# hrz2000/CustomNeRF

Measured on AMD Instinct MI355X. Metric: training rays/s, higher is better.
Workload: dtype f16

## Files before the change

customnerf_amd/_lib.py:

```python
import ctypes as C
import os

import torch

_HERE = os.path.dirname(os.path.abspath(__file__))
LIB_PATH = os.path.join(_HERE, "libcustomnerf_hip.so")
ABI_VERSION = 8

vp, u32, u64, f32, i32 = C.c_void_p, C.c_uint32, C.c_uint64, C.c_float, C.c_int

SIGNATURES = {
    "cnerf_abi_version": [],
    "cnerf_profile_stage_events": [vp, u32],
    "cnerf_near_far_from_aabb": [vp, vp, vp, u32, f32, vp, vp, vp],
    "cnerf_sph_from_ray": [vp, vp, f32, u32, vp, vp],
    "cnerf_morton3D": [vp, u32, vp, vp],
    "cnerf_morton3D_invert": [vp, u32, vp, vp],
    "cnerf_packbits": [vp, u32, f32, vp, vp],
    "cnerf_march_rays_train": [vp, vp, vp, f32, f32, u32, u32, u32, u32, u32, vp, vp, vp, vp, vp, vp, vp, vp, vp],
    "cnerf_march_rays_train_count": [vp, vp, vp, f32, f32, u32, u32, u32, u32, vp, vp, vp, vp, vp, vp],
    "cnerf_march_rays_train_write": [vp, vp, vp, f32, f32, u32, u32, u32, u32, u32, vp, vp, vp, vp, vp, vp, vp, vp],
    "cnerf_march_rays_train_count_hits": [vp, vp, vp, f32, f32, u32, u32, u32, u32, vp, vp, vp, vp, vp, vp, vp],
    "cnerf_march_rays_train_write_hits": [vp, vp, f32, f32, u32, u32, u32, u32, u32, vp, vp, vp, vp, vp, vp, vp, vp],
    "cnerf_composite_rays_train_forward": [vp, vp, vp, vp, u32, u32, f32, vp, vp, vp, u32, vp],
# ... 85 lines not shown
    "cnerf_mesh_atlas_sized_measure": [vp, u32, vp, u32, vp, u64, vp, vp],
    "cnerf_mesh_atlas_sized_layout": [vp, u32, vp, vp, vp],
    "cnerf_mesh_atlas_sized_plan": [u32, u32, u32, vp, vp, u64, vp, vp, u32, vp],
    "cnerf_mesh_atlas_sized_uvs": [u32, u32, vp, vp, vp, u32, vp],
    "cnerf_mesh_atlas_sized_points": [vp, vp, u32, vp, u32, u32, vp, vp, u64, u32, u32, vp, vp, vp, u32, vp],
    "cnerf_mesh_atlas_sized_tspace": [vp, vp, u32, vp, u32, u32, vp, vp, u64, vp, u32, u32, vp, u32, vp, vp, u32, vp],
    "cnerf_mesh_atlas_sized_store": [u32, u32, vp, vp, u64, u32, u32, vp, u32, vp, vp, vp, vp],
    "cnerf_mesh_atlas_sized_fill": [u32, u32, vp, vp, vp],
    "cnerf_mesh_atlas_proj_workspace_bytes": [u32, u32, u32, vp],
    "cnerf_mesh_atlas_proj_charts": [vp, vp, u32, vp, u32, u32, vp, u64, vp, vp, vp, u32, vp, u32, vp],
    "cnerf_mesh_atlas_proj_pack": [vp, u32, u32, u32, vp, vp],
    "cnerf_mesh_atlas_proj_raster": [vp, u32, vp, u32, u32, u32, C.c_double, vp, u32, vp, u64, vp, vp, u32, vp, vp, vp, vp],
    "cnerf_mesh_atlas_proj_points": [vp, vp, u32, vp, u32, u32, vp, u64, u32, u32, vp, vp, vp, u32, vp],
    "cnerf_mesh_atlas_proj_tspace": [vp, vp, u32, vp, u32, u32, vp, u64, vp, u32, u32, vp, u32, vp, vp, u32, vp],
    "cnerf_mesh_atlas_proj_store": [u32, u32, u32, vp, u64, u32, u32, vp, u32, vp, vp, vp],
    "cnerf_mesh_atlas_proj_fill": [u32, u32, u32, vp, u64, vp, vp, vp, vp],
    "cnerf_mesh_tangent_workspace_bytes": [u32, u32, vp],
    "cnerf_mesh_tangent_weld": [vp, vp, u32, u32, vp, u64, vp, vp, u32, vp, u32, vp],
    "cnerf_mesh_tangent_frames": [vp, vp, vp, vp, u32, u32, vp, u64, vp, u32, vp],
    "cnerf_mesh_tangent_vertices": [vp, vp, vp, vp, vp, vp, vp, u32, u32, u32, vp, u64, vp, vp, vp, vp, vp, vp],
    "cnerf_mesh_raster_workspace_bytes": [u32, u32, u32, u32, vp],
    "cnerf_mesh_raster_visibility": [vp, u32, vp, u32, vp, f32, f32, f32, f32, u32, u32, i32, f32, i32, vp, u64, vp, vp, vp, vp, vp],
    "cnerf_mesh_raster_shade": [vp, vp, vp, u32, u32, vp, u32, u32, i32, vp, vp, vp, u32, vp, vp, f32, f32, vp, vp, vp, vp],
    "cnerf_tsdf_integrate": [vp, u32, u32, u32, vp, vp, f32, vp, vp, u32, u32, u32, vp, f32, f32, f32, f32, i32, f32, i32, vp],
    "cnerf_tsdf_finalize": [vp, u32, u32, u32, f32, vp, vp, vp],
    "cnerf_tsdf_face_keep": [vp, u32, u32, u32, vp, vp, vp, u32, vp, u32, vp, vp],
    "cnerf_view_colors_accumulate": [vp, vp, u32, vp, vp, vp, u32, u32, u32, vp, f32, f32, f32, f32, i32, f32, i32, f32, f32, i32, vp, vp, vp],
    "cnerf_view_colors_resolve": [vp, vp, u32, vp, vp, vp, vp, vp],
    "cnerf_mesh_holes_workspace_bytes": [u32, u32, vp],
    "cnerf_mesh_topology": [vp, u32, u32, vp, u64, vp, vp],
    "cnerf_mesh_topology_loops": [u32, u32, vp, u64, vp, u32, vp],
    "cnerf_mesh_holes_count": [vp, u32, u32, u32, vp, u64, vp, vp],
    "cnerf_mesh_holes_emit": [vp, vp, u32, vp, u32, u32, vp, u64, vp, vp, vp, u32, u32, vp],
    "cnerf_mesh_bvh_workspace_bytes": [u32, u32, vp],
    "cnerf_mesh_bvh_build": [vp, u32, vp, u32, vp, u64, vp, vp],
    "cnerf_mesh_bvh_closest": [vp, u64, u32, u32, vp, u32, vp, vp, vp, vp, vp, vp],
    "cnerf_mesh_sample_workspace_bytes": [u32, vp],
    "cnerf_mesh_sample_count": [vp, u32, vp, u32, f32, vp, u64, vp, vp],
    "cnerf_mesh_sample_emit": [vp, u32, vp, u32, f32, vp, u64, vp, vp, vp, vp, u64, vp],
    "cnerf_mesh_bvh_raycast": [vp, u64, u32, u32, vp, vp, u32, f32, f32, vp, vp, i32, vp, vp, vp, vp, vp],
    "cnerf_mesh_bvh_occluded": [vp, u64, u32, u32, vp, vp, u32, f32, f32, vp, vp, i32, vp, vp, vp],
    "cnerf_mesh_bvh_project": [vp, u64, u32, u32, vp, vp, vp, vp, u32, f32, vp, vp, vp, vp, vp, vp, vp, vp],
    "cnerf_mesh_winding_workspace_bytes": [u32, u32, vp],
    "cnerf_mesh_winding_build": [vp, u64, u32, u32, vp, u64, vp],
    "cnerf_mesh_winding_query": [vp, u64, u32, u32, vp, u64, vp, u32, f32, vp, vp, vp],
    "cnerf_mesh_bvh_signed_distance": [vp, u64, u32, u32, vp, u64, vp, u32, f32, vp, vp, vp, vp, vp],
    "cnerf_image_metrics_workspace_bytes": [u32, u32, u32, u32, vp],
    "cnerf_image_metrics": [vp, vp, vp, u32, u32, u32, u32, i32, i32, vp, vp, vp, vp],
    "cnerf_ssim_grad_workspace_bytes": [u32, u32, u32, u32, vp],
    "cnerf_ssim_grad": [vp, vp, vp, u32, u32, u32, u32, i32, vp, vp, vp, vp],
    "cnerf_sd_gemm": [vp, vp, u64, vp],
    "cnerf_sd_gemm_workspace_bytes": [vp, vp],
    "cnerf_sd_gemm_serves_ln": [vp, vp],
    "cnerf_sd_groupnorm_forward": [vp, vp, vp, u32, u32, u32, u32, f32, i32, vp, i32, vp, vp],
    "cnerf_sd_groupnorm_backward": [vp, vp, vp, vp, u32, u32, u32, u32, f32, i32, vp, vp, vp, vp],
    "cnerf_sd_groupnorm_backward_ex": [vp, vp, vp, vp, u32, u32, u32, u32, f32, i32, vp, vp, i32, vp, vp, vp],
    "cnerf_sd_layernorm_forward": [vp, vp, vp, u32, u32, f32, vp, vp],
    "cnerf_sd_softmax_forward": [vp, u64, u32, u32, vp],
    "cnerf_sd_softmax_backward": [vp, vp, u64, u32, u32, vp],
    "cnerf_sd_attention": [vp, vp, vp, vp, u32, u32, u32, u32, u32, u32, u64, u32, u64, u32, u64, u32, u64, i32, vp],
    "cnerf_sd_attention_v": [vp, vp, vp, vp, u32, u32, u32, u32, u32, u32, u64, u32, u64, u32, u64, u32, u64, i32, vp],
    "cnerf_sd_geglu": [vp, u64, u32, vp, vp],
    "cnerf_sd_transpose": [vp, vp, u32, u32, u32, u32, u32, u64, u64, vp],
    "cnerf_sd_image_to_vae_input": [vp, u32, u32, u32, u32, u32, vp, vp],
    "cnerf_sd_image_to_vae_input_backward": [vp, u32, u32, u32, u32, u32, vp, vp],
    "cnerf_sd_clip_preprocess": [vp, u32, u32, u32, u32, vp, vp, vp, vp],
    "cnerf_sd_patchify": [vp, u32, u32, u32, vp, vp],
    "cnerf_sd_timestep_embedding": [vp, u32, u32, vp, vp],
    "cnerf_sd_add_noise": [vp, vp, f32, u32, vp, vp],
    "cnerf_sd_sds_grad": [vp, u32, vp, f32, f32, f32, u32, vp, vp],
    "cnerf_sd_decoder_input": [vp, u32, u32, f32, vp, vp, vp],
    "cnerf_sd_decoder_output": [vp, u32, u32, u32, vp, vp, vp],
    "cnerf_sd_ddim_step": [vp, u32, vp, f32, f32, f32, i32, u32, u32, vp, vp, vp, vp],
    "cnerf_edit_ray_images": [vp, u32, u32, vp, vp, vp, vp],
    "cnerf_edit_ray_images_backward": [vp, vp, vp, u32, u32, vp, vp],
    "cnerf_edit_l1_loss": [vp, vp, u32, f32, vp, vp, vp],
    "cnerf_edit_sds_loss": [vp, vp, u32, vp, vp, vp],
    "cnerf_edit_scale_by_scalar": [vp, vp, f32, u32, vp, vp],
    "cnerf_sd_sample_latents": [vp, vp, u32, u32, f32, vp, vp],
    "cnerf_sd_sample_latents_backward": [vp, vp, vp, u32, u32, f32, vp, vp],
    "cnerf_set_floats": [vp, vp, u32, vp],
    "cnerf_sd_add": [vp, vp, u64, vp, vp],
    "cnerf_sd_silu": [vp, u64, vp, vp],
    "cnerf_sd_concat": [vp, vp, u64, u32, u32, vp, vp],
    "cnerf_sd_concat_gn": [vp, vp, u64, u32, u32, vp, vp, u32, u32, vp],
}


class SdGemmDesc(C.Structure):
    _fields_ = [("A", vp), ("B", vp), ("C", vp), ("C32", vp), ("bias", vp), ("bias_rows", vp), ("residual", vp),
                ("M", u32), ("N", u32), ("K", u32), ("lda", u32), ("ldb", u32), ("ldc", u32), ("ldr", u32),
                ("rows_per_bias_row", u32), ("ld_bias_rows", u32), ("alpha", f32), ("act", C.c_int32), ("batch_outer", u32), ("batch_inner", u32),
                ("sa_o", u64), ("sa_i", u64), ("sb_o", u64), ("sb_i", u64), ("sc_o", u64), ("sc_i", u64),
                ("mode", C.c_int32), ("Cin", u32), ("H_in", u32), ("W_in", u32), ("H_out", u32), ("W_out", u32),
                ("KH", u32), ("KW", u32), ("stride", u32), ("pad_t", u32), ("pad_l", u32), ("ups", u32), ("tstride", u32),
                ("gn_sums", vp), ("gn_groups", u32), ("gn_rows", u32),
                ("ln_out", vp), ("ln_gamma", vp), ("ln_beta", vp), ("ln_eps", f32)]

ADAM_MAX_JOBS = 8


class AdamJobs(C.Structure):
    _fields_ = [("p", vp * ADAM_MAX_JOBS), ("g", vp * ADAM_MAX_JOBS), ("m", vp * ADAM_MAX_JOBS), ("v", vp * ADAM_MAX_JOBS), ("p_half", vp * ADAM_MAX_JOBS),
                ("n", u64 * ADAM_MAX_JOBS), ("lr", f32 * ADAM_MAX_JOBS), ("n_jobs", u32)]


# ... 115 lines not shown
```

customnerf_amd/csrc/sd_gemm.hip:

```cpp
#include "common.h"
#include "../../include/customnerf_sd.h"
#include "sd_gn_fix.h"

typedef _Float16 sd_h8 __attribute__((ext_vector_type(8)));
typedef float sd_f16v __attribute__((ext_vector_type(16)));
typedef float sd_f4 __attribute__((ext_vector_type(4)));

#define SG_BM 128
#define SG_BK 64
#define SG_LDK (SG_BK + 8)
#define SG_THREADS 256

__host__ __device__ __forceinline__ int sg_rho(int r, int hi) { return (r & 3) + 8 * (r >> 2) + 4 * hi; }
__host__ __device__ constexpr uint32_t sg_stage_halfs(int bn) { return (SG_BM + bn) * SG_LDK; }
__host__ __device__ constexpr uint32_t sg_lds_bytes(int bn) {
    const uint32_t stages = 2 * sg_stage_halfs(bn) * 2, ctile = SG_BM * (bn + 4) * 4;
    return stages > ctile ? stages : ctile;
}
__host__ __device__ constexpr uint32_t sg_lds_bytes_glds(int bn) {
    const uint32_t stages = 2 * (SG_BM + bn) * SG_BK * 2, ctile = SG_BM * (bn + 4) * 4;
    return stages > ctile ? stages : ctile;
}

__device__ __forceinline__ float sg_act(float v, int act) {
    if (act == 1) return v * __builtin_amdgcn_rcpf(1.0f + __expf(-v));
    if (act == 2) return 0.5f * v * (1.0f + erff(v * 0.70710678118654752f));
    if (act == 3) return v * __builtin_amdgcn_rcpf(1.0f + __expf(-1.702f * v));
    return v;
}

__device__ __forceinline__ bool sg_coord(int32_t num, uint32_t tstride, uint32_t ups, uint32_t n_in, uint32_t &out) {
    if (num < 0) return false;
    if (tstride == 2) {
        if (num & 1) return false;
        num >>= 1;
    }
    if (ups == 2) num >>= 1;
    out = (uint32_t)num;
    return out < n_in;
}

template <int BM, int BN, int NTHREADS, bool SPLIT>
__device__ __forceinline__ void sg_epilogue_phase2(const CnerfSdGemm &g, const float *ct, long long (*gn_lds)[36][2], uint32_t tid, uint32_t m0, uint32_t n0,
                                                   uint32_t zo, uint32_t zi, uint32_t split, float *__restrict__ partial) {
    constexpr uint32_t LDC = BN + 4;
    constexpr int SG_EPI_THREADS = NTHREADS;
    const bool do_gn = !SPLIT && g.gn_sums != nullptr;
    constexpr int GI = 4;
    const uint32_t gn_cg = do_gn ? g.N / g.gn_groups : 1u;
    const uint32_t gn_g0 = n0 / gn_cg, gn_i0 = do_gn ? m0 / g.gn_rows : 0u;
    if (do_gn) {
        for (uint32_t i = tid; i < GI * 36 * 2; i += SG_EPI_THREADS) (&gn_lds[0][0][0])[i] = 0;
        __syncthreads();
    }
    float gs[2][2] = {{0.0f, 0.0f}, {0.0f, 0.0f}};
// ... 122 lines not shown
            if (full && ((g.ldc | n) & 7) == 0 && ((((uintptr_t)C) & 15) == 0)) {
                sd_h8 o;
#pragma unroll
                for (int e = 0; e < 8; e++) o[e] = (_Float16)v[e];
                *reinterpret_cast<sd_h8 *>(cp) = o;
            } else {
#pragma unroll
                for (int e = 0; e < 8; e++)
                    if (INSIDE || n + e < g.N) cp[e] = (_Float16)v[e];
            }
        }
        if (C32) {
            float *cp = C32 + (size_t)m * ldc32 + n;
#pragma unroll
            for (int e = 0; e < 8; e++)
                if (INSIDE || n + e < g.N) cp[e] = v[e];
        }
    }
    };
    const bool inside = m0 + BM <= g.M && n0 + BN <= g.N;
    if (!gn3) {
        if (inside) phase2(std::true_type{}, std::false_type{});
        else phase2(std::false_type{}, std::false_type{});
    } else phase2(std::false_type{}, std::true_type{});
    if (do_gn) {
        if (gn_img != 0xFFFFFFFFu) {
            const uint32_t gl = (n0 + (tid % CPR) * 8) / gn_cg - gn_g0;
            gn_add(&gn_lds[gn_img - gn_i0][gl][0], gs[0][0]);
            gn_add(&gn_lds[gn_img - gn_i0][gl][1], gs[0][1]);
            gn_add(&gn_lds[gn_img - gn_i0][gl + 1][0], gs[1][0]);
            gn_add(&gn_lds[gn_img - gn_i0][gl + 1][1], gs[1][1]);
            if (gn3) {
                gn_add(&gn_lds[gn_img - gn_i0][gl + 2][0], gs3[0]);
                gn_add(&gn_lds[gn_img - gn_i0][gl + 2][1], gs3[1]);
            }
        }
        __syncthreads();
        const uint32_t n_img = g.M / g.gn_rows;
        for (uint32_t i = tid; i < GI * 36; i += SG_EPI_THREADS) {
            const uint32_t im = i / 36, gl = i % 36, img = gn_i0 + im, grp = gn_g0 + gl;
            const long long a = gn_lds[im][gl][0], b2 = gn_lds[im][gl][1];
            if (img < n_img && grp < g.gn_groups) {
                long long *dst = reinterpret_cast<long long *>(g.gn_sums) + ((size_t)img * g.gn_groups + grp) * 2;
                gn_add_fixed(dst, a);
                gn_add_fixed(dst + 1, b2);
            }
        }
    }
}

__device__ __forceinline__ uint32_t sg_swz(uint32_t row, uint32_t chunk) { return chunk ^ ((row >> 1) & 7u); }

template <int AMODE, int NT, bool SPLIT, bool GLDS = false, bool SIMPLE = false>
__global__ void __launch_bounds__(SG_THREADS) k_sd_gemm(const CnerfSdGemm g, float *__restrict__ partial, uint32_t k_tiles_per_split) {
    constexpr int BN = 64 * NT;
    constexpr int MT = 2, BM = SG_BM;
    constexpr int CB = BN * 8 / SG_THREADS;
    constexpr uint32_t STAGE = sg_stage_halfs(BN);
    extern __shared__ __attribute__((aligned(16))) unsigned char sg_lds[];
    _Float16 *lds = reinterpret_cast<_Float16 *>(sg_lds);
    const uint32_t tid = threadIdx.x, lane = tid & 63, wave = tid >> 6, hi = lane >> 5, li = lane & 31;
    const uint32_t wm = wave >> 1, wn = wave & 1;
    const uint32_t m0 = blockIdx.x * BM, n0 = blockIdx.y * BN;
    uint32_t z = 0, split = 0;
    if (SPLIT) split = blockIdx.z; else z = blockIdx.z;
    const uint32_t zo = z / g.batch_inner, zi = z - zo * g.batch_inner;
    const _Float16 *A = reinterpret_cast<const _Float16 *>(g.A) + g.sa_o * zo + g.sa_i * zi;
    const _Float16 *B = reinterpret_cast<const _Float16 *>(g.B) + g.sb_o * zo + g.sb_i * zi;

    const uint32_t arow = tid >> 1, ak = (tid & 1) * 32;
    const uint32_t brow = tid / (8 / CB), bk = (tid % (8 / CB)) * CB * 8;
    const _Float16 *abase;
    int32_t oh_s = 0, ow_s = 0;
    bool a_valid;
    {
        const uint32_t m = m0 + arow;
        a_valid = m < g.M;
        if (AMODE == 0) abase = A + (size_t)m * g.lda;
        else {
            const uint32_t hw = g.H_out * g.W_out;
            const uint32_t img = m / hw, rem = m - img * hw, oh = rem / g.W_out, ow = rem - oh * g.W_out;
            abase = A + (size_t)img * g.H_in * g.W_in * g.Cin;
            oh_s = (int32_t)(oh * g.stride) - (int32_t)g.pad_t;
            ow_s = (int32_t)(ow * g.stride) - (int32_t)g.pad_l;
        }
    }
    const uint32_t nrow = n0 + brow;
    const bool b_valid = nrow < g.N;
    const _Float16 *bbase = B + (size_t)nrow * g.ldb;

    const uint32_t n_ktiles = (g.K + SG_BK - 1) / SG_BK;
    uint32_t kt0 = 0, kt1 = n_ktiles;
    if (SPLIT) { kt0 = split * k_tiles_per_split; kt1 = min(kt0 + k_tiles_per_split, n_ktiles); }

    uint32_t t_kh = 0, t_kw = 0, t_c0 = 0;
    if (AMODE == 2) {
        const uint32_t tap = (kt0 * SG_BK) / g.Cin;
        t_c0 = kt0 * SG_BK - tap * g.Cin;
        t_kh = tap / g.KW;
        t_kw = tap - t_kh * g.KW;
    }

    sd_f16v acc[MT][NT];
#pragma unroll
    for (int i = 0; i < MT; i++)
#pragma unroll
        for (int j = 0; j < NT; j++)
#pragma unroll
            for (int r = 0; r < 16; r++) acc[i][j][r] = 0.0f;

    if constexpr (!GLDS) {
        uint4 sa[4], sb[CB];
        auto fetch = [&](uint32_t kt) __attribute__((always_inline)) {
            const uint32_t k = kt * SG_BK;
            if (AMODE == 0) {
    #pragma unroll
                for (int c = 0; c < 4; c++) sa[c] = (a_valid && k + ak + 8 * c < g.K) ? *reinterpret_cast<const uint4 *>(abase + k + ak + 8 * c) : make_uint4(0, 0, 0, 0);
            } else if (AMODE == 2) {
// ... 38 lines not shown
        __syncthreads();
        for (uint32_t kt = kt0; kt < kt1; kt++) {
            const uint32_t stage = (kt - kt0) & 1;
            if (kt + 1 < kt1) fetch(kt + 1);
            const _Float16 *sA = lds + stage * STAGE, *sB = sA + SG_BM * SG_LDK;
    #pragma unroll
            for (int s = 0; s < SG_BK / 16; s++) {
                sd_h8 a[2], b[NT];
    #pragma unroll
                for (int i = 0; i < 2; i++) a[i] = *reinterpret_cast<const sd_h8 *>(sA + (wm * 64 + i * 32 + li) * SG_LDK + s * 16 + 8 * hi);
    #pragma unroll
                for (int j = 0; j < NT; j++) b[j] = *reinterpret_cast<const sd_h8 *>(sB + (wn * 32 * NT + j * 32 + li) * SG_LDK + s * 16 + 8 * hi);
    #pragma unroll
                for (int i = 0; i < 2; i++)
    #pragma unroll
                    for (int j = 0; j < NT; j++) acc[i][j] = __builtin_amdgcn_mfma_f32_32x32x16_f16(a[i], b[j], acc[i][j], 0, 0, 0);
            }
            if (kt + 1 < kt1) commit(stage ^ 1);
            __syncthreads();
        }


    } else {
        constexpr uint32_t GSTAGE = (BM + BN) * SG_BK * 2;
        constexpr int RA = BM / 32;
        constexpr int RB = BN / 32;
        const uint32_t grow = tid >> 3, gch = tid & 7u;
        constexpr uint32_t OOB = 0xFFFFFF00u;
        const uint32_t a_batch = AMODE == 0 ? 1u : g.M / (g.H_out * g.W_out);
        const uint32_t a_bytes = AMODE == 0 ? (uint32_t)(((size_t)(g.M - 1) * g.lda + g.K) * 2) : (uint32_t)((size_t)a_batch * g.H_in * g.W_in * g.Cin * 2);
        const uint32_t b_bytes = (uint32_t)(((size_t)(g.N - 1) * g.ldb + g.K) * 2);
        const __amdgpu_buffer_rsrc_t rsA = __builtin_amdgcn_make_buffer_rsrc(const_cast<_Float16 *>(A), 0, a_bytes, 0x00020000);
        const __amdgpu_buffer_rsrc_t rsB = __builtin_amdgcn_make_buffer_rsrc(const_cast<_Float16 *>(B), 0, b_bytes, 0x00020000);
        constexpr bool simple = SIMPLE;
        const uint32_t wave_u = __builtin_amdgcn_readfirstlane(wave);
        uint32_t a_off[RA];
        int32_t a_oh[RA], a_ow[RA];
        bool a_ok[RA];
        const uint32_t a_sc0 = sg_swz(grow, gch) * 8;
#pragma unroll
        for (int r = 0; r < RA; r++) {
            const uint32_t row = 32 * r + grow, m = m0 + row;
            a_ok[r] = m < g.M;
            a_oh[r] = a_ow[r] = 0;
            const uint32_t mm = a_ok[r] ? m : 0;
            if (AMODE == 0) a_off[r] = (mm * g.lda + a_sc0) * 2;
            else {
                const uint32_t hw = g.H_out * g.W_out;
                const uint32_t img = mm / hw, rem = mm - img * hw, oh = rem / g.W_out, ow = rem - oh * g.W_out;
                a_oh[r] = (int32_t)(oh * g.stride) - (int32_t)g.pad_t;
                a_ow[r] = (int32_t)(ow * g.stride) - (int32_t)g.pad_l;
                a_off[r] = ((img * g.H_in + (uint32_t)a_oh[r]) * g.W_in + (uint32_t)a_ow[r]) * g.Cin * 2 + a_sc0 * 2;
                if (!simple) a_off[r] = img * g.H_in * g.W_in * g.Cin * 2 + a_sc0 * 2;
            }
        }
        uint32_t b_off[RB];
#pragma unroll
        for (int r = 0; r < RB; r++) {
            const uint32_t row = 32 * r + grow, n = n0 + row;
            b_off[r] = n < g.N ? (n * g.ldb + sg_swz(row, gch) * 8) * 2 : OOB;
        }
        uint32_t i_k = 0, i_tap = 0;
        unsigned char *i_sA = sg_lds, *i_sB = sg_lds;
        bool i_kin = true;
        auto issue_begin = [&](uint32_t kt, uint32_t stage) __attribute__((always_inline)) {
            i_k = kt * SG_BK;
            i_sA = sg_lds + (size_t)stage * GSTAGE;
            i_sB = i_sA + BM * SG_BK * 2;
            i_kin = i_k + a_sc0 < g.K;
            i_tap = AMODE == 2 ? ((t_kh * g.W_in + t_kw) * g.Cin + t_c0) * 2 : i_k * 2;
        };
        auto issue_round = [&](int q) __attribute__((always_inline)) {
            if (q < RA) {
                const int r = q;
                uint32_t voff;
                if (AMODE == 0) {
                    voff = (a_off[r] + i_tap) | ((a_ok[r] && i_kin) ? 0u : OOB);
                } else if (simple) {
                    const bool ok = a_ok[r] && (uint32_t)(a_oh[r] + (int32_t)t_kh) < g.H_in && (uint32_t)(a_ow[r] + (int32_t)t_kw) < g.W_in;
                    voff = (a_off[r] + i_tap) | (ok ? 0u : OOB);
                } else {
                    uint32_t ih = 0, iw = 0;
                    const bool ok = a_ok[r] && sg_coord(a_oh[r] + (int32_t)t_kh, g.tstride, g.ups, g.H_in, ih) &&
                                    sg_coord(a_ow[r] + (int32_t)t_kw, g.tstride, g.ups, g.W_in, iw);
                    voff = ok ? a_off[r] + ((ih * g.W_in + iw) * g.Cin + t_c0) * 2 : OOB;
                }
                __builtin_amdgcn_raw_ptr_buffer_load_lds(rsA, (__attribute__((address_space(3))) void *)(i_sA + (32 * r + 8 * wave_u) * 128), 16, voff, 0, 0, 0);
            } else {
                const int r = q - RA;
                const uint32_t voff = b_off[r] | (i_kin ? 0u : OOB);
                __builtin_amdgcn_raw_ptr_buffer_load_lds(rsB, (__attribute__((address_space(3))) void *)(i_sB + (32 * r + 8 * wave_u) * 128), 16, voff, i_k * 2, 0, 0);
            }
        };
        auto issue_end = [&]() __attribute__((always_inline)) {
            if (AMODE == 2) {
                t_c0 += SG_BK;
                if (t_c0 >= g.Cin) {
                    t_c0 = 0;
                    if (++t_kw == g.KW) { t_kw = 0; ++t_kh; }
                }
            }
        };
        auto issue = [&](uint32_t kt, uint32_t stage) __attribute__((always_inline)) {
            issue_begin(kt, stage);
#pragma unroll
            for (int q = 0; q < RA + RB; q++) issue_round(q);
            issue_end();
        };
        uint32_t a_rd[MT][4], b_rd[NT][4];
#pragma unroll
        for (int s2 = 0; s2 < 4; s2++) {
#pragma unroll
            for (int i = 0; i < MT; i++) {
                const uint32_t row = wm * 32 * MT + i * 32 + li;
                a_rd[i][s2] = row * 128 + sg_swz(row, 2 * s2 + hi) * 16;
            }
#pragma unroll
            for (int j = 0; j < NT; j++) {
                const uint32_t row = wn * 32 * NT + j * 32 + li;
                b_rd[j][s2] = row * 128 + sg_swz(row, 2 * s2 + hi) * 16;
            }
        }
        if (kt0 < kt1) issue(kt0, 0);
        asm volatile("s_waitcnt vmcnt(0)" ::: "memory");
        __syncthreads();
        for (uint32_t kt = kt0; kt < kt1; kt++) {
            const uint32_t stage = (kt - kt0) & 1;
            if (kt + 1 < kt1) issue(kt + 1, stage ^ 1);
            const unsigned char *sA = sg_lds + (size_t)stage * GSTAGE, *sB = sA + BM * SG_BK * 2;
            sd_h8 a[2][MT], b[2][NT];
// ... 399 lines not shown
        }
    }
    const float mean = cn_wave_sum(sum) / (float)g.N;
    float sq = 0.0f;
#pragma unroll
    for (int c = 0; c < CPL; c++)
        if (lane + 64 * c < nchunks) {
#pragma unroll
            for (int e = 0; e < 8; e++) { const float d = v[c][e] - mean; sq += d * d; }
        }
    const float rstd = rsqrtf(cn_wave_sum(sq) / (float)g.N + g.ln_eps);
#pragma unroll
    for (int c = 0; c < CPL; c++) {
        const uint32_t col = lane + 64 * c;
        if (col < nchunks) {
            sd_h8 o;
#pragma unroll
            for (int e = 0; e < 8; e++) o[e] = (_Float16)((v[c][e] - mean) * rstd * g.ln_gamma[col * 8 + e] + g.ln_beta[col * 8 + e]);
            *reinterpret_cast<sd_h8 *>(reinterpret_cast<_Float16 *>(g.ln_out) + (size_t)m * g.N + col * 8) = o;
        }
    }
}

static bool sg_ln_admissible(const CnerfSdGemm *g) {
    return g->ln_out && g->ln_gamma && g->ln_beta && g->C && !g->C32 && !g->gn_sums && g->act != 4 && (g->N & 7) == 0 && g->N <= 2048 && (g->ldc & 7) == 0 &&
           (!g->residual || (g->ldr & 7) == 0) && g->batch_outer * g->batch_inner == 1 &&
           ((((uintptr_t)g->C) | ((uintptr_t)g->ln_out) | ((uintptr_t)g->residual)) & 15) == 0;
}

static int sg_check(const CnerfSdGemm *g) {
    if (!g) return CNERF_ENULL;
    if (!g->A || !g->B || (!g->C && !g->C32)) return CNERF_ENULL;
    if (g->M == 0 || g->N == 0 || g->K == 0 || (g->K & 7) || (g->ldb & 7)) return CNERF_EINVAL;
    if (g->batch_outer == 0 || g->batch_inner == 0) return CNERF_EINVAL;
    if (g->act < 0 || g->act > 4) return CNERF_EINVAL;
    if (g->act == 4 && ((g->N & 7) || g->residual || g->C32 || !g->C || g->gn_sums)) return CNERF_EINVAL;
    if (g->bias_rows && g->rows_per_bias_row == 0) return CNERF_EINVAL;
    if (g->gn_sums && (g->gn_groups == 0 || g->N % g->gn_groups || g->N / g->gn_groups < 4 || g->gn_rows < 64 || g->M % g->gn_rows ||
                       g->batch_outer * g->batch_inner != 1))
        return CNERF_EINVAL;
    if ((((uintptr_t)g->A) | ((uintptr_t)g->B)) & 15) return CNERF_EINVAL;
    if (g->mode == 0) {
        if (g->lda & 7) return CNERF_EINVAL;
    } else if (g->mode == 1) {
        if (g->Cin == 0 || (g->Cin & 7) || g->KH == 0 || g->KW == 0 || g->K != g->KH * g->KW * g->Cin) return CNERF_EINVAL;
        if (g->H_out == 0 || g->W_out == 0 || g->M % (g->H_out * g->W_out)) return CNERF_EINVAL;
        if (g->ups < 1 || g->ups > 2 || g->tstride < 1 || g->tstride > 2 || g->stride == 0) return CNERF_EINVAL;
        if (g->batch_outer * g->batch_inner != 1) return CNERF_EINVAL;
    } else return CNERF_EINVAL;
    return CNERF_OK;
}

struct SgPlan { int nt; uint32_t splits, kps; };
static int sg_env(const char *name) { return cn_tune_env(name, 0); }
static SgPlan sg_plan(const CnerfSdGemm *g) {
    const uint32_t n_ktiles = cn_div_up(g->K, SG_BK);
    const uint32_t batch = g->batch_outer * g->batch_inner;
    static const int force_nt = sg_env("CNERF_SG_NT"), force_sp = sg_env("CNERF_SG_SPLITS");
    SgPlan best = {1, 1, n_ktiles};
    double best_cost = 1e30;
    for (int nt = 1; nt <= 2; nt++) {
        if (force_nt && nt != force_nt) continue;
        const uint32_t tiles = cn_div_up(g->M, SG_BM) * cn_div_up(g->N, 64 * nt) * batch;
        const double t_k = nt == 1 ? 1.0 : 1.5;
        const uint32_t max_sp = batch != 1 ? 1 : 32;
        for (uint32_t sp = 1; sp <= max_sp; sp++) {
            if (force_sp && sp != (uint32_t)force_sp && !(batch != 1 && sp == 1)) continue;
            const uint32_t kps = cn_div_up(n_ktiles, sp);
            if (sp > 1 && (kps < 8 || cn_div_up(n_ktiles, kps) != sp)) continue;
            const uint64_t blocks = (uint64_t)tiles * sp;
            const double rounds = (double)((blocks + 511) / 512);
            double cost = rounds * (kps + 8.0) * t_k;
            if (blocks < 256) cost *= 0.6 + 0.4 * (double)blocks / 256.0;
            if (sp > 1) cost += 3.0 + 2.0 * (double)g->M * g->N * 4.0 * sp / 4.0e6;
            if (cost < best_cost) { best_cost = cost; best = {nt, sp, kps}; }
        }
    }
    return best;
}
static int sg_pick_nt(const CnerfSdGemm *g) { return sg_plan(g).nt; }
static uint32_t sg_splits(const CnerfSdGemm *g, int nt, uint32_t &k_tiles_per_split) {
    (void)nt;
    const SgPlan p = sg_plan(g);
    k_tiles_per_split = p.kps;
    return p.splits;
}

static bool sg_glds_fits(const CnerfSdGemm *g) {
    const uint64_t lim = 0xFFFFFF00ull - 4096;
    const uint64_t a_bytes = g->mode == 0 ? ((uint64_t)(g->M - 1) * g->lda + g->K) * 2
                                          : (uint64_t)(g->M / (g->H_out * g->W_out)) * g->H_in * g->W_in * g->Cin * 2;
    const uint64_t b_bytes = ((uint64_t)(g->N - 1) * g->ldb + g->K) * 2;
    return a_bytes < lim && b_bytes < lim;
}
static bool sg_use_glds(const CnerfSdGemm *g) {
    static const int v = cn_tune_env("CNERF_SG_GLDS", 1);
    return v != 0 && sg_glds_fits(g);
}

#ifdef CNERF_TUNING
static bool sg_use_big(const CnerfSdGemm *g, const SgPlan &plan) {
    static const int on = cn_tune_env("CNERF_SG_BIG", 0);
    static const int min_tiles = cn_tune_env("CNERF_SG_BIG_TILES", 224), min_k = cn_tune_env("CNERF_SG_BIG_K", 512);
    if (!on || plan.splits > 1 || !sg_use_glds(g)) return false;
    if (g->mode != 0 && (g->Cin % SG_BK) != 0) return false;
    if (g->gn_sums && g->gn_rows < 128) return false;
    if (g->K < (uint32_t)min_k || (g->N % SGB_BN) > 0 && (g->N % SGB_BN) <= 64 && g->N < 1024) return false;
    const uint64_t tiles = (uint64_t)cn_div_up(g->M, SGB_BM) * cn_div_up(g->N, SGB_BN) * g->batch_outer * g->batch_inner;
    return tiles >= (uint64_t)min_tiles;
}

template <int SCHED>
static void sgb_launch_s(const CnerfSdGemm *g, hipStream_t st) {
    const dim3 grid(cn_div_up(g->M, SGB_BM), cn_div_up(g->N, SGB_BN), g->batch_outer * g->batch_inner);
    static bool attr_set = false;
    if (!attr_set) {
        (void)hipFuncSetAttribute(reinterpret_cast<const void *>(&k_sd_gemm_big<0, false, SCHED>), hipFuncAttributeMaxDynamicSharedMemorySize, sgb_lds_bytes());
        (void)hipFuncSetAttribute(reinterpret_cast<const void *>(&k_sd_gemm_big<2, false, SCHED>), hipFuncAttributeMaxDynamicSharedMemorySize, sgb_lds_bytes());
        (void)hipFuncSetAttribute(reinterpret_cast<const void *>(&k_sd_gemm_big<2, true, SCHED>), hipFuncAttributeMaxDynamicSharedMemorySize, sgb_lds_bytes());
        attr_set = true;
    }
    if (g->mode == 0) hipLaunchKernelGGL((k_sd_gemm_big<0, false, SCHED>), grid, dim3(SGB_THREADS), sgb_lds_bytes(), st, *g);
    else if (g->tstride == 1 && g->ups == 1) hipLaunchKernelGGL((k_sd_gemm_big<2, true, SCHED>), grid, dim3(SGB_THREADS), sgb_lds_bytes(), st, *g);
    else hipLaunchKernelGGL((k_sd_gemm_big<2, false, SCHED>), grid, dim3(SGB_THREADS), sgb_lds_bytes(), st, *g);
}
static void sgb_launch(const CnerfSdGemm *g, hipStream_t st) {
    static const int sched = cn_tune_env("CNERF_SGB_SCHED", 2);
    if (sched == 0) { sgb_launch_s<0>(g, st); return; }
    if (sched == 1) { sgb_launch_s<1>(g, st); return; }
    sgb_launch_s<2>(g, st);
}
#endif

template <int AMODE, int NT, bool SPLIT, bool GLDS, bool SIMPLE = false>
static void sg_launch_g(const CnerfSdGemm *g, dim3 grid, hipStream_t st, float *partial, uint32_t kps) {
    if constexpr (GLDS && AMODE == 2 && !SIMPLE) {
        if (g->tstride == 1 && g->ups == 1) { sg_launch_g<AMODE, NT, SPLIT, GLDS, true>(g, grid, st, partial, kps); return; }
    }
    static bool attr_set = false;
    auto kern = k_sd_gemm<AMODE, NT, SPLIT, GLDS, SIMPLE>;
    const uint32_t lds_bytes = GLDS ? sg_lds_bytes_glds(64 * NT) : sg_lds_bytes(64 * NT);
    if (!attr_set) {
        (void)hipFuncSetAttribute(reinterpret_cast<const void *>(kern), hipFuncAttributeMaxDynamicSharedMemorySize, lds_bytes);
        attr_set = true;
    }
    hipLaunchKernelGGL(kern, grid, dim3(SG_THREADS), lds_bytes, st, *g, partial, kps);
}

template <int AMODE, int NT, bool SPLIT>
static void sg_launch(const CnerfSdGemm *g, dim3 grid, hipStream_t st, float *partial, uint32_t kps) {
    if constexpr (AMODE != 1) {
        if (sg_use_glds(g)) { sg_launch_g<AMODE, NT, SPLIT, true>(g, grid, st, partial, kps); return; }
    }
    static bool attr_set = false;
    auto kern = k_sd_gemm<AMODE, NT, SPLIT, false>;
    const uint32_t lds_bytes = sg_lds_bytes(64 * NT);
    if (!attr_set) {
        (void)hipFuncSetAttribute(reinterpret_cast<const void *>(kern), hipFuncAttributeMaxDynamicSharedMemorySize, lds_bytes);
        attr_set = true;
    }
    hipLaunchKernelGGL(kern, grid, dim3(SG_THREADS), lds_bytes, st, *g, partial, kps);
}

template <int AMODE>
static void sg_launch_nt(const CnerfSdGemm *g, int nt, bool split, dim3 grid, hipStream_t st, float *partial, uint32_t kps) {
    if (nt == 2) {
        if (split) sg_launch<AMODE, 2, true>(g, grid, st, partial, kps); else sg_launch<AMODE, 2, false>(g, grid, st, partial, kps);
    } else {
        if (split) sg_launch<AMODE, 1, true>(g, grid, st, partial, kps); else sg_launch<AMODE, 1, false>(g, grid, st, partial, kps);
    }
}

extern "C" {

int cnerf_sd_gemm_workspace_bytes(const CnerfSdGemm *g, uint64_t *bytes) {
    if (!bytes) return CNERF_ENULL;
    int rc = sg_check(g);
    if (rc) return rc;
    uint32_t kps;
    const uint32_t splits = sg_splits(g, sg_pick_nt(g), kps);
    *bytes = splits > 1 ? (uint64_t)splits * g->M * g->N * sizeof(float) : 0;
    return CNERF_OK;
}

int cnerf_sd_gemm(const CnerfSdGemm *g, void *workspace, uint64_t workspace_bytes, void *stream) {
    int rc = sg_check(g);
    if (rc) return rc;
    hipStream_t st = CN_STREAM(stream);
    const SgPlan plan = sg_plan(g);
    const int nt = plan.nt;
    uint32_t kps = plan.kps;
    uint32_t splits = plan.splits;
    if (splits > 1 && (!workspace || workspace_bytes < (uint64_t)splits * g->M * g->N * sizeof(float))) {
        splits = 1;
        kps = cn_div_up(g->K, SG_BK);
    }
    if (splits > 1 && g->gn_sums && (uint64_t)(g->M / g->gn_rows) * g->gn_groups > SG_EPI_GN_MAX) {
        splits = 1;
        kps = cn_div_up(g->K, SG_BK);
    }
    const bool split = splits > 1;
#ifdef CNERF_TUNING
    if (!split && sg_use_big(g, plan)) {
        sgb_launch(g, st);
        return cn_launch_status();
    }
#endif
    const dim3 grid(cn_div_up(g->M, SG_BM), cn_div_up(g->N, 64 * nt), split ? splits : g->batch_outer * g->batch_inner);
    const int amode = g->mode == 0 ? 0 : ((g->Cin % SG_BK) == 0 ? 2 : 1);
    float *partial = reinterpret_cast<float *>(workspace);
    if (amode == 0) sg_launch_nt<0>(g, nt, split, grid, st, partial, kps);
    else if (amode == 1) sg_launch_nt<1>(g, nt, split, grid, st, partial, kps);
    else sg_launch_nt<2>(g, nt, split, grid, st, partial, kps);
    if (split && sg_ln_admissible(g)) {
        const dim3 eg(cn_div_up(g->M, 4));
        const float *pw = reinterpret_cast<const float *>(workspace);
        const uint32_t cpl = cn_div_up(g->N / 8, 64);
        if (cpl == 1) hipLaunchKernelGGL(k_sd_gemm_splitk_epilogue_ln<1>, eg, dim3(256), 0, st, *g, pw, splits);
        else if (cpl == 2) hipLaunchKernelGGL(k_sd_gemm_splitk_epilogue_ln<2>, eg, dim3(256), 0, st, *g, pw, splits);
        else hipLaunchKernelGGL(k_sd_gemm_splitk_epilogue_ln<4>, eg, dim3(256), 0, st, *g, pw, splits);
    } else if (split) {
        const size_t total = (size_t)g->M * g->N;
        uint32_t eb = (uint32_t)((total + 255) / 256 > 2048 ? 2048 : (total + 255) / 256);
        if (g->gn_sums) {
            const uint32_t n_slabs = (g->gn_groups & 3u) == 0 ? g->gn_groups / 4 : 1u;
            uint32_t row_chunks = cn_div_up(eb, n_slabs);
            if (row_chunks > g->M) row_chunks = g->M;
            eb = n_slabs * (row_chunks ? row_chunks : 1u);
        }
        hipLaunchKernelGGL(k_sd_gemm_splitk_epilogue, dim3(eb), dim3(256), 0, st, *g, reinterpret_cast<const float *>(workspace), splits);
    }
    return cn_launch_status();
}

int cnerf_sd_gemm_serves_ln(const CnerfSdGemm *g, int *yes) {
    if (!yes) return CNERF_ENULL;
    *yes = 0;
    int rc = sg_check(g);
    if (rc) return rc;
    uint32_t splits = sg_plan(g).splits;
    if (splits > 1 && g->gn_sums && (uint64_t)(g->M / g->gn_rows) * g->gn_groups > SG_EPI_GN_MAX) splits = 1;
    *yes = (splits > 1 && sg_ln_admissible(g)) ? 1 : 0;
    return CNERF_OK;
}

}
```

customnerf_amd/sd/ops.py:

```python
import ctypes

import torch

from .._lib import lib, check, ptr, stream, require_cuda, SdGemmDesc, query_u64, ScratchCache

ACT_NONE, ACT_SILU, ACT_GELU, ACT_QUICK_GELU, ACT_GEGLU = 0, 1, 2, 3, 4
TAIL_FUSION = True
_PROFILE = None


def set_profile(records):
    global _PROFILE
    _PROFILE = records


_WS = ScratchCache(floor=64 << 20, retire=True)
_WS_RETIRED = _WS.retired


def _workspace(nbytes, device):
    return _WS.reserve(device, int(nbytes), device)


def _launch(d, device):
    need = query_u64(lib.cnerf_sd_gemm_workspace_bytes, ctypes.byref(d))
    ws = _workspace(need, device) if need else None
    if not TAIL_FUSION and need:
        d.gn_sums = None
    if _PROFILE is not None:
        e0, e1 = torch.cuda.Event(enable_timing=True), torch.cuda.Event(enable_timing=True)
        e0.record()
    check(lib.cnerf_sd_gemm(ctypes.byref(d), ptr(ws), ws.numel() if ws is not None else 0, stream()), "sd_gemm")
    if _PROFILE is not None:
        e1.record()
        _PROFILE.append((e0, e1, 2.0 * d.M * d.N * d.K * d.batch_outer * d.batch_inner, (int(d.M), int(d.N), int(d.K), int(d.mode), int(d.batch_outer * d.batch_inner), int(d.H_in), int(d.Cin), int(d.tstride), int(d.ups))))
    return need > 0


def _attach_gn(d, gn, M, N):
    if gn is None:
        return False
    sums, groups, rows = gn
    if rows < 64 or M % rows or N % groups or N // groups < 4:
        return False
    d.gn_sums, d.gn_groups, d.gn_rows = ptr(sums), groups, rows
    return True


def _desc(A, B, C, M, N, K, lda, ldb, ldc, bias=None, bias_rows=None, rows_per_bias_row=0, residual=None, ldr=0, act=0, alpha=1.0, C32=None):
    d = SdGemmDesc()
    d.A, d.B, d.C, d.C32 = ptr(A), ptr(B), ptr(C), ptr(C32)
    d.bias, d.bias_rows, d.residual = ptr(bias), ptr(bias_rows), ptr(residual)
    d.M, d.N, d.K, d.lda, d.ldb, d.ldc, d.ldr = M, N, K, lda, ldb, ldc, ldr
    d.rows_per_bias_row, d.alpha, d.act = rows_per_bias_row, alpha, act
    d.batch_outer = d.batch_inner = 1
    d.ups = d.tstride = 1
    return d


def linear(x, w, bias=None, residual=None, act=ACT_NONE, alpha=1.0, out=None, out32=False, gn=None, ln=None):
    require_cuda(x, w)
    K = x.shape[-1]
    N = w.shape[0]
    x2 = x.reshape(-1, K)
    M = x2.shape[0]
    assert w.shape[1] == K and x2.stride(1) == 1 and x2.dtype == torch.float16 and w.dtype == torch.float16
# ... 412 lines not shown
```

include/customnerf_sd.h:

```cpp
#ifndef CUSTOMNERF_SD_H
#define CUSTOMNERF_SD_H

#include <stdint.h>

#ifdef __cplusplus
extern "C" {
#endif

typedef struct CnerfSdGemm {
    const void *A;
    const void *B;
    void *C;
    float *C32;
    const float *bias;
    const float *bias_rows;
    const void *residual;
    uint32_t M, N, K;
    uint32_t lda, ldb, ldc, ldr;
    uint32_t rows_per_bias_row;
    uint32_t ld_bias_rows;
    float alpha;
    int32_t act;
    uint32_t batch_outer, batch_inner;
    uint64_t sa_o, sa_i, sb_o, sb_i, sc_o, sc_i;
    int32_t mode;
    uint32_t Cin, H_in, W_in, H_out, W_out, KH, KW, stride, pad_t, pad_l, ups, tstride;
    int64_t *gn_sums;
    uint32_t gn_groups, gn_rows;
    void *ln_out;
    const float *ln_gamma, *ln_beta;
    float ln_eps;
} CnerfSdGemm;

int cnerf_sd_gemm(const CnerfSdGemm *desc, void *workspace, uint64_t workspace_bytes, void *stream);
int cnerf_sd_gemm_workspace_bytes(const CnerfSdGemm *desc, uint64_t *bytes);
int cnerf_sd_gemm_serves_ln(const CnerfSdGemm *desc, int *yes);

#define CNERF_SD_GN_FRAC_BITS 20
int cnerf_sd_groupnorm_forward(const void *x, const float *gamma, const float *beta, uint32_t B, uint32_t HW, uint32_t C,
                               uint32_t G, float eps, int silu, int64_t *sums, int zero_sums, void *y, void *stream);
int cnerf_sd_groupnorm_backward(const void *x, const void *dy, const float *gamma, const float *beta, uint32_t B, uint32_t HW,
                                uint32_t C, uint32_t G, float eps, int silu, const int64_t *sums, int64_t *scratch, void *dx,
                                void *stream);
int cnerf_sd_groupnorm_backward_ex(const void *x, const void *dy, const float *gamma, const float *beta, uint32_t B, uint32_t HW,
                                   uint32_t C, uint32_t G, float eps, int silu, const int64_t *sums, int64_t *scratch,
                                   int scratch_is_zero, const void *residual, void *dx, void *stream);

int cnerf_sd_layernorm_forward(const void *x, const float *gamma, const float *beta, uint32_t rows, uint32_t C, float eps,
                               void *y, void *stream);

int cnerf_sd_softmax_forward(void *S, uint64_t rows, uint32_t cols, uint32_t ld, void *stream);
int cnerf_sd_softmax_backward(const void *P, void *dP, uint64_t rows, uint32_t cols, uint32_t ld, void *stream);

int cnerf_sd_attention(const void *q, const void *k, const void *vT, void *out, uint32_t B, uint32_t H, uint32_t Tq, uint32_t Tk,
                       uint32_t d, uint32_t ldq, uint64_t sq, uint32_t ldk, uint64_t sk, uint32_t ldv, uint64_t sv, uint32_t ldo,
                       uint64_t so, int causal, void *stream);
int cnerf_sd_attention_v(const void *q, const void *k, const void *v, void *out, uint32_t B, uint32_t H, uint32_t Tq, uint32_t Tk,
                         uint32_t d, uint32_t ldq, uint64_t sq, uint32_t ldk, uint64_t sk, uint32_t ldv, uint64_t sv, uint32_t ldo,
                         uint64_t so, int causal, void *stream);

int cnerf_sd_geglu(const void *x, uint64_t rows, uint32_t C, void *y, void *stream);

int cnerf_sd_transpose(const void *src, void *dst, uint32_t rows, uint32_t cols, uint32_t lds, uint32_t ldd, uint32_t batch,
                       uint64_t ss, uint64_t sd, void *stream);

int cnerf_sd_image_to_vae_input(const float *img, uint32_t B, uint32_t Hi, uint32_t Wi, uint32_t Ho, uint32_t Wo, void *out,
                                void *stream);
int cnerf_sd_image_to_vae_input_backward(const void *d_out, uint32_t B, uint32_t Hi, uint32_t Wi, uint32_t Ho, uint32_t Wo,
                                         float *d_img, void *stream);

int cnerf_sd_clip_preprocess(const float *img, uint32_t B, uint32_t Hi, uint32_t Wi, uint32_t S, const float *mean3, const float *std3,
                             float *out, void *stream);
int cnerf_sd_patchify(const float *x, uint32_t B, uint32_t S, uint32_t P, void *out, void *stream);

int cnerf_sd_timestep_embedding(const float *t, uint32_t B, uint32_t dim, void *out, void *stream);

int cnerf_sd_add_noise(const float *latents, const float *noise, float alpha_bar, uint32_t pixels, void *unet_in, void *stream);
int cnerf_sd_sds_grad(const void *eps, uint32_t ld_eps, const float *noise, float alpha_bar, float guidance, float lambda_sd,
                      uint32_t pixels, float *grad, void *stream);

int cnerf_sd_decoder_input(const float *latents, uint32_t B, uint32_t hw, float scaling_factor, const float *post_quant, void *out,
                           void *stream);
int cnerf_sd_decoder_output(const void *x, uint32_t ld, uint32_t B, uint32_t HW, float *img, uint8_t *img_u8, void *stream);
int cnerf_sd_ddim_step(const void *eps, uint32_t ld_eps, const float *latents, float alpha_bar_t, float alpha_bar_prev, float guidance,
                       int mode, uint32_t pairs, uint32_t pixels, float *latents_out, float *x0_out, void *unet_in, void *stream);

int cnerf_sd_add(const void *a, const void *b, uint64_t n, void *y, void *stream);
int cnerf_sd_silu(const void *x, uint64_t n, void *y, void *stream);
int cnerf_sd_concat(const void *a, const void *b, uint64_t rows, uint32_t C1, uint32_t C2, void *y, void *stream);
// ... 20 lines not shown
```

Before: 8.843 million.

## Add XCD-aware tile ordering and direct-to-LDS loader for Cin=8 convolutions

```diff
diff --git a/customnerf_amd/_lib.py b/customnerf_amd/_lib.py
--- a/customnerf_amd/_lib.py
+++ b/customnerf_amd/_lib.py
@@ -161,6 +161,8 @@
     "cnerf_sd_gemm": [vp, vp, u64, vp],
     "cnerf_sd_gemm_workspace_bytes": [vp, vp],
     "cnerf_sd_gemm_serves_ln": [vp, vp],
+    "cnerf_sd_gemm_set_tile_order": [i32],
+    "cnerf_sd_gemm_set_cin8_loader": [i32],
     "cnerf_sd_groupnorm_forward": [vp, vp, vp, u32, u32, u32, u32, f32, i32, vp, i32, vp, vp],
     "cnerf_sd_groupnorm_backward": [vp, vp, vp, vp, u32, u32, u32, u32, f32, i32, vp, vp, vp, vp],
     "cnerf_sd_groupnorm_backward_ex": [vp, vp, vp, vp, u32, u32, u32, u32, f32, i32, vp, vp, i32, vp, vp, vp],
diff --git a/customnerf_amd/csrc/sd_gemm.hip b/customnerf_amd/csrc/sd_gemm.hip
--- a/customnerf_amd/csrc/sd_gemm.hip
+++ b/customnerf_amd/csrc/sd_gemm.hip
@@ -1,6 +1,10 @@
 #include "common.h"
 #include "../../include/customnerf_sd.h"
 #include "sd_gn_fix.h"
+#include "sd_gemm_tile_order.h"
+#include <atomic>
+
+#define SG_TILE_ORDER_DEFAULT 1
 
 typedef _Float16 sd_h8 __attribute__((ext_vector_type(8)));
 typedef float sd_f16v __attribute__((ext_vector_type(16)));
@@ -229,7 +233,8 @@
 __device__ __forceinline__ uint32_t sg_swz(uint32_t row, uint32_t chunk) { return chunk ^ ((row >> 1) & 7u); }
 
 template <int AMODE, int NT, bool SPLIT, bool GLDS = false, bool SIMPLE = false>
-__global__ void __launch_bounds__(SG_THREADS) k_sd_gemm(const CnerfSdGemm g, float *__restrict__ partial, uint32_t k_tiles_per_split) {
+__global__ void __launch_bounds__(SG_THREADS) k_sd_gemm(const CnerfSdGemm g, float *__restrict__ partial, uint32_t k_tiles_per_split,
+                                                        uint32_t tiles_m, uint32_t tiles_n, int order) {
     constexpr int BN = 64 * NT;
     constexpr int MT = 2, BM = SG_BM;
     constexpr int CB = BN * 8 / SG_THREADS;
@@ -238,9 +243,12 @@
     _Float16 *lds = reinterpret_cast<_Float16 *>(sg_lds);
     const uint32_t tid = threadIdx.x, lane = tid & 63, wave = tid >> 6, hi = lane >> 5, li = lane & 31;
     const uint32_t wm = wave >> 1, wn = wave & 1;
-    const uint32_t m0 = blockIdx.x * BM, n0 = blockIdx.y * BN;
+    SgTile tile = {blockIdx.x, blockIdx.y, blockIdx.z};
+    if (!SPLIT && order != 0) tile = sg_tile_of(blockIdx.x, tiles_m, tiles_n, gridDim.x / (tiles_m * tiles_n), 1);
+    const uint32_t m0 = __builtin_amdgcn_readfirstlane(tile.mt) * BM, n0 = __builtin_amdgcn_readfirstlane(tile.nt) * BN;
+    const uint32_t tz = __builtin_amdgcn_readfirstlane(tile.z);
     uint32_t z = 0, split = 0;
-    if (SPLIT) split = blockIdx.z; else z = blockIdx.z;
+    if (SPLIT) split = tz; else z = tz;
     const uint32_t zo = z / g.batch_inner, zi = z - zo * g.batch_inner;
     const _Float16 *A = reinterpret_cast<const _Float16 *>(g.A) + g.sa_o * zo + g.sa_i * zi;
     const _Float16 *B = reinterpret_cast<const _Float16 *>(g.B) + g.sb_o * zo + g.sb_i * zi;
@@ -385,6 +393,7 @@
                 a_ow[r] = (int32_t)(ow * g.stride) - (int32_t)g.pad_l;
                 a_off[r] = ((img * g.H_in + (uint32_t)a_oh[r]) * g.W_in + (uint32_t)a_ow[r]) * g.Cin * 2 + a_sc0 * 2;
                 if (!simple) a_off[r] = img * g.H_in * g.W_in * g.Cin * 2 + a_sc0 * 2;
+                if (AMODE == 3) a_off[r] = img * g.H_in * g.W_in * 16;
             }
         }
         uint32_t b_off[RB];
@@ -393,7 +402,7 @@
             const uint32_t row = 32 * r + grow, n = n0 + row;
             b_off[r] = n < g.N ? (n * g.ldb + sg_swz(row, gch) * 8) * 2 : OOB;
         }
-        uint32_t i_k = 0, i_tap = 0;
+        uint32_t i_k = 0, i_tap = 0, i_kh = 0, i_kw = 0;
         unsigned char *i_sA = sg_lds, *i_sB = sg_lds;
         bool i_kin = true;
         auto issue_begin = [&](uint32_t kt, uint32_t stage) __attribute__((always_inline)) {
@@ -402,6 +411,11 @@
             i_sB = i_sA + BM * SG_BK * 2;
             i_kin = i_k + a_sc0 < g.K;
             i_tap = AMODE == 2 ? ((t_kh * g.W_in + t_kw) * g.Cin + t_c0) * 2 : i_k * 2;
+            if (AMODE == 3) {
+                const uint32_t tap = (i_k + a_sc0) >> 3;
+                i_kh = tap / g.KW;
+                i_kw = tap - i_kh * g.KW;
+            }
         };
         auto issue_round = [&](int q) __attribute__((always_inline)) {
             if (q < RA) {
@@ -409,6 +423,11 @@
                 uint32_t voff;
                 if (AMODE == 0) {
                     voff = (a_off[r] + i_tap) | ((a_ok[r] && i_kin) ? 0u : OOB);
+                } else if (AMODE == 3) {
+                    uint32_t ih = 0, iw = 0;
+                    const bool ok = a_ok[r] && i_kin && sg_coord(a_oh[r] + (int32_t)i_kh, g.tstride, g.ups, g.H_in, ih) &&
+                                    sg_coord(a_ow[r] + (int32_t)i_kw, g.tstride, g.ups, g.W_in, iw);
+                    voff = (a_off[r] + (ih * g.W_in + iw) * 16) | (ok ? 0u : OOB);
                 } else if (simple) {
                     const bool ok = a_ok[r] && (uint32_t)(a_oh[r] + (int32_t)t_kh) < g.H_in && (uint32_t)(a_ow[r] + (int32_t)t_kw) < g.W_in;
                     voff = (a_off[r] + i_tap) | (ok ? 0u : OOB);
@@ -914,6 +933,8 @@
 }
 
 struct SgPlan { int nt; uint32_t splits, kps; };
+struct SgGrid { uint32_t tiles_m, tiles_n, zc; int order; };
+static dim3 sg_dim3(const SgGrid &g) { return g.order ? dim3(g.tiles_m * g.tiles_n * g.zc) : dim3(g.tiles_m, g.tiles_n, g.zc); }
 static int sg_env(const char *name) { return cn_tune_env(name, 0); }
 static SgPlan sg_plan(const CnerfSdGemm *g) {
     const uint32_t n_ktiles = cn_div_up(g->K, SG_BK);
@@ -960,6 +981,23 @@
     return v != 0 && sg_glds_fits(g);
 }
 
+static std::atomic<int> g_sg_cin8_dma{1};
+static int sg_amode(const CnerfSdGemm *g) {
+    if (g->mode == 0) return 0;
+    if ((g->Cin % SG_BK) == 0) return 2;
+    if (g->Cin == 8 && g_sg_cin8_dma.load(std::memory_order_relaxed) && sg_use_glds(g)) return 3;
+    return 1;
+}
+
+static std::atomic<int> g_sg_tile_order{SG_TILE_ORDER_DEFAULT};
+static int sg_tile_order(const CnerfSdGemm *g, const SgGrid &grid, bool split) {
+    if (split || !g_sg_tile_order.load(std::memory_order_relaxed)) return 0;
+    if (g_sg_tile_order.load(std::memory_order_relaxed) == 2) return 1;
+    if (grid.tiles_n < 2 || grid.tiles_m < 64 || (uint64_t)grid.tiles_m * grid.tiles_n * grid.zc <= 512) return 0;
+    if (g->mode != 0 && (g->tstride != 1 || g->ups != 1)) return 0;
+    return 1;
+}
+
 #ifdef CNERF_TUNING
 static bool sg_use_big(const CnerfSdGemm *g, const SgPlan &plan) {
     static const int on = cn_tune_env("CNERF_SG_BIG", 0);
@@ -995,7 +1033,7 @@
 #endif
 
 template <int AMODE, int NT, bool SPLIT, bool GLDS, bool SIMPLE = false>
-static void sg_launch_g(const CnerfSdGemm *g, dim3 grid, hipStream_t st, float *partial, uint32_t kps) {
+static void sg_launch_g(const CnerfSdGemm *g, SgGrid grid, hipStream_t st, float *partial, uint32_t kps) {
     if constexpr (GLDS && AMODE == 2 && !SIMPLE) {
         if (g->tstride == 1 && g->ups == 1) { sg_launch_g<AMODE, NT, SPLIT, GLDS, true>(g, grid, st, partial, kps); return; }
     }
@@ -1006,26 +1044,31 @@
         (void)hipFuncSetAttribute(reinterpret_cast<const void *>(kern), hipFuncAttributeMaxDynamicSharedMemorySize, lds_bytes);
         attr_set = true;
     }
-    hipLaunchKernelGGL(kern, grid, dim3(SG_THREADS), lds_bytes, st, *g, partial, kps);
+    hipLaunchKernelGGL(kern, sg_dim3(grid), dim3(SG_THREADS), lds_bytes, st, *g, partial, kps, grid.tiles_m, grid.tiles_n, grid.order);
 }
 
 template <int AMODE, int NT, bool SPLIT>
-static void sg_launch(const CnerfSdGemm *g, dim3 grid, hipStream_t st, float *partial, uint32_t kps) {
-    if constexpr (AMODE != 1) {
-        if (sg_use_glds(g)) { sg_launch_g<AMODE, NT, SPLIT, true>(g, grid, st, partial, kps); return; }
-    }
-    static bool attr_set = false;
-    auto kern = k_sd_gemm<AMODE, NT, SPLIT, false>;
-    const uint32_t lds_bytes = sg_lds_bytes(64 * NT);
-    if (!attr_set) {
-        (void)hipFuncSetAttribute(reinterpret_cast<const void *>(kern), hipFuncAttributeMaxDynamicSharedMemorySize, lds_bytes);
-        attr_set = true;
-    }
-    hipLaunchKernelGGL(kern, grid, dim3(SG_THREADS), lds_bytes, st, *g, partial, kps);
+static void sg_launch(const CnerfSdGemm *g, SgGrid grid, hipStream_t st, float *partial, uint32_t kps) {
+    if constexpr (AMODE == 3) {
+        sg_launch_g<AMODE, NT, SPLIT, true>(g, grid, st, partial, kps);
+        return;
+    } else {
+        if constexpr (AMODE != 1) {
+            if (sg_use_glds(g)) { sg_launch_g<AMODE, NT, SPLIT, true>(g, grid, st, partial, kps); return; }
+        }
+        static bool attr_set = false;
+        auto kern = k_sd_gemm<AMODE, NT, SPLIT, false>;
+        const uint32_t lds_bytes = sg_lds_bytes(64 * NT);
+        if (!attr_set) {
+            (void)hipFuncSetAttribute(reinterpret_cast<const void *>(kern), hipFuncAttributeMaxDynamicSharedMemorySize, lds_bytes);
+            attr_set = true;
+        }
+        hipLaunchKernelGGL(kern, sg_dim3(grid), dim3(SG_THREADS), lds_bytes, st, *g, partial, kps, grid.tiles_m, grid.tiles_n, grid.order);
+    }
 }
 
 template <int AMODE>
-static void sg_launch_nt(const CnerfSdGemm *g, int nt, bool split, dim3 grid, hipStream_t st, float *partial, uint32_t kps) {
+static void sg_launch_nt(const CnerfSdGemm *g, int nt, bool split, SgGrid grid, hipStream_t st, float *partial, uint32_t kps) {
     if (nt == 2) {
         if (split) sg_launch<AMODE, 2, true>(g, grid, st, partial, kps); else sg_launch<AMODE, 2, false>(g, grid, st, partial, kps);
     } else {
@@ -1068,12 +1111,14 @@
         return cn_launch_status();
     }
 #endif
-    const dim3 grid(cn_div_up(g->M, SG_BM), cn_div_up(g->N, 64 * nt), split ? splits : g->batch_outer * g->batch_inner);
-    const int amode = g->mode == 0 ? 0 : ((g->Cin % SG_BK) == 0 ? 2 : 1);
+    const SgGrid grid = {cn_div_up(g->M, SG_BM), cn_div_up(g->N, 64 * nt), split ? splits : g->batch_outer * g->batch_inner, 0};
+    const SgGrid ordered = {grid.tiles_m, grid.tiles_n, grid.zc, sg_tile_order(g, grid, split)};
+    const int amode = sg_amode(g);
     float *partial = reinterpret_cast<float *>(workspace);
-    if (amode == 0) sg_launch_nt<0>(g, nt, split, grid, st, partial, kps);
-    else if (amode == 1) sg_launch_nt<1>(g, nt, split, grid, st, partial, kps);
-    else sg_launch_nt<2>(g, nt, split, grid, st, partial, kps);
+    if (amode == 0) sg_launch_nt<0>(g, nt, split, ordered, st, partial, kps);
+    else if (amode == 1) sg_launch_nt<1>(g, nt, split, ordered, st, partial, kps);
+    else if (amode == 3) sg_launch_nt<3>(g, nt, split, ordered, st, partial, kps);
+    else sg_launch_nt<2>(g, nt, split, ordered, st, partial, kps);
     if (split && sg_ln_admissible(g)) {
         const dim3 eg(cn_div_up(g->M, 4));
         const float *pw = reinterpret_cast<const float *>(workspace);
@@ -1095,6 +1140,18 @@
     return cn_launch_status();
 }
 
+int cnerf_sd_gemm_set_tile_order(int order) {
+    if (order < 0 || order > 2) return CNERF_EINVAL;
+    g_sg_tile_order.store(order, std::memory_order_relaxed);
+    return CNERF_OK;
+}
+
+int cnerf_sd_gemm_set_cin8_loader(int dma) {
+    if (dma != 0 && dma != 1) return CNERF_EINVAL;
+    g_sg_cin8_dma.store(dma, std::memory_order_relaxed);
+    return CNERF_OK;
+}
+
 int cnerf_sd_gemm_serves_ln(const CnerfSdGemm *g, int *yes) {
     if (!yes) return CNERF_ENULL;
     *yes = 0;
diff --git a/customnerf_amd/csrc/sd_gemm_tile_order.h b/customnerf_amd/csrc/sd_gemm_tile_order.h
--- /dev/null
+++ b/customnerf_amd/csrc/sd_gemm_tile_order.h
@@ -0,0 +1,32 @@
+#pragma once
+#include <stdint.h>
+
+#if defined(__HIPCC__) || defined(__CUDACC__)
+#define SG_TILE_HD __host__ __device__
+#else
+#define SG_TILE_HD
+#endif
+
+#define SG_TILE_NXCD 8u
+
+struct SgTile { uint32_t mt, nt, z; };
+
+SG_TILE_HD inline SgTile sg_tile_of(uint32_t lin, uint32_t tiles_m, uint32_t tiles_n, uint32_t batch, int order) {
+    SgTile t;
+    if (order == 0) {
+        t.mt = lin % tiles_m;
+        const uint32_t rest = lin / tiles_m;
+        t.nt = rest % tiles_n;
+        t.z = rest / tiles_n;
+        return t;
+    }
+    const uint32_t n = tiles_m * tiles_n * batch, q = n / SG_TILE_NXCD, r = n % SG_TILE_NXCD;
+    const uint32_t xcd = lin % SG_TILE_NXCD, k = lin / SG_TILE_NXCD;
+    const uint32_t pos = (xcd < r ? xcd * (q + 1) : r * (q + 1) + (xcd - r) * q) + k;
+    const uint32_t per_z = tiles_m * tiles_n;
+    t.z = pos / per_z;
+    const uint32_t rem = pos - t.z * per_z;
+    t.mt = rem / tiles_n;
+    t.nt = rem - t.mt * tiles_n;
+    return t;
+}
diff --git a/customnerf_amd/sd/ops.py b/customnerf_amd/sd/ops.py
--- a/customnerf_amd/sd/ops.py
+++ b/customnerf_amd/sd/ops.py
@@ -12,6 +12,14 @@
 def set_profile(records):
     global _PROFILE
     _PROFILE = records
+
+
+def set_tile_order(order):
+    check(lib.cnerf_sd_gemm_set_tile_order(int(order)), "sd_gemm_set_tile_order")
+
+
+def set_cin8_loader(dma):
+    check(lib.cnerf_sd_gemm_set_cin8_loader(int(dma)), "sd_gemm_set_cin8_loader")
 
 
 _WS = ScratchCache(floor=64 << 20, retire=True)
diff --git a/include/customnerf_sd.h b/include/customnerf_sd.h
--- a/include/customnerf_sd.h
+++ b/include/customnerf_sd.h
@@ -35,6 +35,8 @@
 int cnerf_sd_gemm(const CnerfSdGemm *desc, void *workspace, uint64_t workspace_bytes, void *stream);
 int cnerf_sd_gemm_workspace_bytes(const CnerfSdGemm *desc, uint64_t *bytes);
 int cnerf_sd_gemm_serves_ln(const CnerfSdGemm *desc, int *yes);
+int cnerf_sd_gemm_set_tile_order(int order);
+int cnerf_sd_gemm_set_cin8_loader(int dma);
 
 #define CNERF_SD_GN_FRAC_BITS 20
 int cnerf_sd_groupnorm_forward(const void *x, const float *gamma, const float *beta, uint32_t B, uint32_t HW, uint32_t C,
```

Measured after the change: 8.872 million (median of 6 runs). No clear change (+0.3%).
